# biagiom/spark-network-traffic-classifier

Hardware: NVIDIA H100
Metric: flow-records/sec fit+transform (higher is better)
Workload: dtype u8 bins / uint32 histograms / f64 split scoring (f32 records)

## Files before the change

include/b200flow.h:

```cpp
#ifndef B200FLOW_H
#define B200FLOW_H

#include <stdint.h>

#ifdef __cplusplus
extern "C" {
#endif

#define B200FLOW_OK            0
#define B200FLOW_ERR_ARG      -1
#define B200FLOW_ERR_CUDA     -2
#define B200FLOW_ERR_LIMIT    -3

#define B200FLOW_F32 0
#define B200FLOW_F64 1

#define B200FLOW_SRC_F32    0
#define B200FLOW_SRC_F64    1
#define B200FLOW_SRC_I32    2
#define B200FLOW_SRC_INDEX  3
#define B200FLOW_SRC_ONEHOT 4

typedef struct b200flow_slot {
    int32_t kind;
// ... 114 lines not shown
                        const uint32_t* node_counts, const uint32_t* left_counts,
                        const uint32_t* right_counts, int32_t C,
                        b200flow_node* nodes, uint64_t* node_mask, uint32_t* pool_counts,
                        int32_t* node_tree, int64_t pool_capacity,
                        int32_t* next_tree, uint32_t* next_nid, int32_t* next_node,
                        int32_t* next_parent, int32_t* child_slot, int64_t* counters, void* stream);

int b200flow_partition_level(const uint8_t* tp, int32_t tp_stride,
                             const void* ent, void* ent_out,
                             int32_t n_slots, const int64_t* seg_begin, const int64_t* seg_end,
                             const int64_t* chunk_off, int64_t n_chunks, int32_t chunk_rows,
                             const b200flow_split* split, int32_t* cursors, void* stream);

int b200flow_route_hist_config(int32_t F, int32_t m, int32_t n_bins, int32_t C,
                               int32_t rec_bytes , int32_t* chunk_rows, int32_t* m_pass);
int b200flow_route_hist_level(const uint8_t* tp, int32_t tp_stride, int32_t F,
                              const int32_t* field_desc ,
                              const void* ent, void* ent_out,
                              int32_t n_slots, const int64_t* seg_begin, const int64_t* seg_end,
                              const int64_t* chunk_off, const int64_t* n_chunks_dev ,
                              int64_t n_chunks_max ,
                              int32_t chunk_rows,
                              const b200flow_split* split, const int32_t* child_slot, int32_t* cursors,
                              void* chunk_scratch ,
                              const uint16_t* subset_next, int32_t m, int32_t n_bins, int32_t C,
                              uint32_t* hist_next, int32_t flags, void* stream);

int b200flow_packed_layout(int32_t F, const int32_t* feat_bins, int32_t C, int32_t* desc, int32_t* rec_bytes);
int b200flow_pack_records(const uint8_t* tp, int32_t tp_stride, int64_t n_rows, int32_t F, const int32_t* desc,
                          int32_t rec_bytes, uint32_t* packed, void* stream);

int b200flow_plan_route(int32_t n_slots, const b200flow_split* split, const int64_t* seg_begin, const int64_t* seg_end,
                        int32_t chunk_rows, const int32_t* slot_node, double* node_gain, int32_t* n_chunks,
                        int32_t* cursors , void* stream);

int b200flow_next_segments(int32_t n_next , const int64_t* n_next_dev ,
                           const int32_t* next_parent,
                           const int64_t* seg_begin, const int64_t* seg_end,
                           const int32_t* cursors, int64_t* next_begin, int64_t* next_end,
                           void* stream);

int b200flow_finalize_forest(int64_t n_nodes, const uint32_t* pool_counts, int32_t C,
                             double* leaf_prob, void* stream);

int b200flow_predict(const uint8_t* tp, int32_t tp_stride, int64_t n_rows,
                     const b200flow_node* nodes, const uint64_t* node_mask,
                     const double* leaf_prob, const uint32_t* pool_counts,
                     int32_t T, int32_t C, int32_t dt_mode,
                     const void* top_nodes , int32_t top_levels,
                     double* raw, double* prob, double* pred, void* stream);

int b200flow_build_top_nodes(const b200flow_node* nodes, const int32_t* node_tree, int64_t n_nodes, int32_t T,
                             int32_t top_levels, void* top, void* stream);

int b200flow_gather_rows(const void* src, int32_t row_bytes, const int32_t* idx, int64_t n_rows, void* out, void* stream);

int b200flow_confusion(const double* pred, const double* label, int64_t n_rows, int32_t C,
                       int64_t* cm, void* stream);

int b200flow_predict_grid_confusion(const uint8_t* tp, int32_t tp_stride, int32_t F, int64_t n_rows, const int32_t* mult,
                                    const b200flow_node* nodes, const uint64_t* node_mask, const double* leaf_prob,
                                    const uint32_t* pool_counts, int32_t T, int32_t C, int32_t dt_mode,
                                    const void* top_nodes, int32_t top_levels, const int32_t* tree_cuts_host,
                                    int32_t n_tree_cuts, const int32_t* depth_cuts_host, int32_t n_depth_cuts,
                                    int32_t cm_side, int32_t max_depth_cuts_per_launch, int64_t* cm, void* stream);
int b200flow_predict_grid_scores(const uint8_t* tp, int32_t tp_stride, int32_t F, int64_t n_rows,
                                 const b200flow_node* nodes, const uint64_t* node_mask, const double* leaf_prob,
                                 const uint32_t* pool_counts, int32_t T, int32_t C, int32_t dt_mode,
                                 const void* top_nodes, int32_t top_levels, const int32_t* tree_cuts_host,
                                 int32_t n_tree_cuts, const int32_t* depth_cuts_host, int32_t n_depth_cuts,
                                 int32_t max_depth_cuts_per_launch, double* scores, void* stream);

int b200flow_binary_counts_scratch(int32_t S, int64_t n, int64_t* scratch_bytes);
int b200flow_binary_counts(const double* scores, int64_t score_stride, const int32_t* pos, const int32_t* neg,
                           int64_t count_stride, int32_t S, int64_t n, void* scratch, int64_t scratch_bytes,
                           double* d_score, int64_t* d_pos, int64_t* d_neg, int64_t cap, int64_t* n_distinct,
                           int64_t* n_nan, void* stream);
int b200flow_binary_curve(const double* d_score, const int64_t* d_pos, const int64_t* d_neg, int64_t cap,
                          const int64_t* n_distinct, int32_t S, int32_t num_bins, double* auc, double* c_score,
                          int64_t* c_tp, int64_t* c_fp, int64_t* c_n, double* work, void* stream);

int b200flow_kmeans_assign(const double* x, int64_t n_rows, int32_t D, int64_t ld, const double* centers, int32_t k,
                           int32_t* cluster, double* dist, void* stream);
int b200flow_group_sums_chunks(int64_t row_offset, int64_t n_rows, int64_t* n_chunks);
int b200flow_group_sums(const double* values, int64_t ld, const int32_t* ids, int64_t n_rows, int32_t W, int32_t G,
                        int64_t row_offset, double* partials, int64_t* counts, void* stream);
int b200flow_group_sums_chain(const double* partials, int64_t n_chunks, int32_t G, int32_t W, double* totals, void* stream);
int b200flow_kmeans_row_keys(uint64_t seed, int64_t row_offset, int64_t n_rows, int64_t* keys, void* stream);
int b200flow_kmeans_select(uint64_t seed, int64_t row_offset, int64_t n_rows, int32_t step, const double* cost, int32_t k,
                           double sum_cost, uint8_t* flag, void* stream);
int b200flow_silhouette_rows(const double* x, int64_t n_rows, int32_t D, int64_t ld, const double* norms, const int32_t* cluster,
                             const double* Y, const double* psi, const int64_t* N, int32_t G, double* out, void* stream);

int b200flow_mlp_config(const int32_t* layers, int32_t n_layers, int64_t* n_params, int64_t* smem_bytes);
int b200flow_mlp_loss_grad(const void* x, int32_t x_dtype, int64_t n_rows, int64_t ld, const int32_t* labels,
                           const int32_t* layers, int32_t n_layers, const double* weights, int64_t row_offset,
                           double* partials, void* stream);
int b200flow_mlp_forward(const void* x, int32_t x_dtype, int64_t n_rows, int64_t ld, const int32_t* layers, int32_t n_layers,
                         const double* weights, double* raw, void* stream);

int b200flow_svc_config(int32_t D, int64_t K, int32_t* block_classes, int32_t* class_blocks, int64_t* smem_bytes);
int b200flow_svc_loss_grad(const void* x, int32_t x_dtype, int64_t n_rows, int64_t ld, int32_t D, const int32_t* labels,
                           const int32_t* positives, int64_t K, const double* inv_std, const double* weights,
                           int64_t row_offset, double* partials, void* stream);
int b200flow_svc_margins(const void* x, int32_t x_dtype, int64_t n_rows, int64_t ld, int32_t D, int64_t K,
                         const double* weights, double* raw, void* stream);
// ... 152 lines not shown
```

spark-network-traffic-classifier_b200/b200flow/_lib.py:

```python
import ctypes as C
import os

import numpy as np
import torch

_HERE = os.path.dirname(os.path.abspath(__file__))
LIB_PATH = os.path.join(_HERE, "libb200flow.so")

F32, F64 = 0, 1
SRC_F32, SRC_F64, SRC_I32, SRC_INDEX, SRC_ONEHOT = 0, 1, 2, 3, 4

SLOT_DTYPE = np.dtype([("kind", "<i4"), ("src_off", "<i4"), ("lut_off", "<i4"), ("lut_len", "<i4"),
                       ("hot", "<i4"), ("reserved", "<i4"), ("mean", "<f8"), ("scale", "<f8")])
SPLIT_DTYPE = np.dtype([("feat", "<i4"), ("kind", "<i4"), ("bin_thr", "<i4"), ("flags", "<i4"),
                        ("gain", "<f8"), ("impurity", "<f8"), ("mask", "<u8", (4,))])
NODE_DTYPE = np.dtype([("feat", "<i4"), ("kind_bin", "<i4"), ("left", "<i4"), ("nid", "<u4")])
assert SLOT_DTYPE.itemsize == 40 and SPLIT_DTYPE.itemsize == 64 and NODE_DTYPE.itemsize == 16


class B200FlowError(RuntimeError):
    pass


class UnsupportedParamError(B200FlowError, ValueError):
    """a parameter value MLlib accepts but the CUDA path does not implement (entropy impurity, maxBins > 256, ...): a
    ValueError, so the pyspark shim reports it as IllegalArgumentException; CUDA/runtime failures stay B200FlowError."""


_P, _I32, _I64, _U64, _F64 = C.c_void_p, C.c_int32, C.c_int64, C.c_uint64, C.c_double

_SIGNATURES = {
    "b200flow_category_counts": [_P, _I64, _I32, _I32, _I32, _P, _P],
    "b200flow_category_counts_multi": [_P, _I64, _I32, _I32, _P, _P, _P, _P],
    "b200flow_encode": [_P, _I64, _I32, _P, _I32, _P, _I32, _I32, _I32, _I32, _I32, _P, _I32, _P, _P, _P],
    "b200flow_sample_records": [_P, _I64, _I32, _P, _I32, _P, _I32, _U64, _U64, _I64, _P, _I64, _P, _P],
    "b200flow_encode_bins": [_P, _I64, _I32, _P, _I32, _P, _I32, _I32, _I32, _I32, _I32, _I32, _I32, _P, _P, _P, _I32, _P, _I32, _P, _P, _P],
    "b200flow_column_moments": [_P, _I32, _I64, _I32, _I64, _P, _P, _P, _P],
    "b200flow_sample_rows": [_P, _I32, _I64, _I32, _I64, _U64, _U64, _I64, _P, _I64, _P, _P],
    "b200flow_find_splits": [_P, _I64, _I32, _I32, _P, _I32, _P, _P, _P, _P],
    "b200flow_bin_rows": [_P, _I32, _I64, _I32, _I64, _P, _P, _P, _I32, _P, _P, _I32, _P, _P],
    "b200flow_dedup_rows": [_P, _I64, _I32, _I32, _P, _P, _I64, _P, _P, _P, _P, _P, _P, _P, _P],
    "b200flow_bag_weights": [_U64, _I32, _I64, _I64, _P, _P, _P, _P, _I64, _P, _P],
    "b200flow_group_rows": [_P, _I64, _I64, _P, _P, _P, _P, _P, _P],
    "b200flow_bag_count": [_P, _I32, _I64, _P, _P],
    "b200flow_bag_fill": [_P, _I32, _I64, _P, _P, _P],
    "b200flow_exclusive_scan_i32_to_i64": [_P, _I64, _P, _P, _P],
    "b200flow_feature_subsets": [_U64, _I32, _P, _P, _I32, _I32, _P, _P],
    "b200flow_hist_level": [_P, _I32, _I32, _P, _I32, _P, _P, _P, _I64, _I32, _P, _I32, _I32, _I32, _P, _P],
    "b200flow_score_level": [_P, _I32, _P, _I32, _I32, _I32, _P, _P, _I32, _I32, _I32, _F64, _P, _P, _P, _P, _P],
    "b200flow_grow_level": [_I32, _P, _P, _P, _P, _P, _P, _P, _I32, _P, _P, _P, _P, _I64, _P, _P, _P, _P, _P, _P, _P],
    "b200flow_route_hist_level": [_P, _I32, _I32, _P, _P, _P, _I32, _P, _P, _P, _P, _I64, _I32, _P, _P, _P, _P, _P, _I32, _I32,
                                  _I32, _P, _I32, _P],
    "b200flow_pack_records": [_P, _I32, _I64, _I32, _P, _I32, _P, _P],
    "b200flow_partition_level": [_P, _I32, _P, _P, _I32, _P, _P, _P, _I64, _I32, _P, _P, _P],
    "b200flow_plan_route": [_I32, _P, _P, _P, _I32, _P, _P, _P, _P, _P],
    "b200flow_next_segments": [_I32, _P, _P, _P, _P, _P, _P, _P, _P],
    "b200flow_finalize_forest": [_I64, _P, _I32, _P, _P],
    "b200flow_predict": [_P, _I32, _I64, _P, _P, _P, _P, _I32, _I32, _I32, _P, _I32, _P, _P, _P, _P],
    "b200flow_build_top_nodes": [_P, _P, _I64, _I32, _I32, _P, _P],
    "b200flow_gather_rows": [_P, _I32, _P, _I64, _P, _P],
    "b200flow_confusion": [_P, _P, _I64, _I32, _P, _P],
    "b200flow_predict_grid_confusion": [_P, _I32, _I32, _I64, _P, _P, _P, _P, _P, _I32, _I32, _I32, _P, _I32, _P, _I32, _P, _I32,
                                        _I32, _I32, _P, _P],
    "b200flow_predict_grid_scores": [_P, _I32, _I32, _I64, _P, _P, _P, _P, _I32, _I32, _I32, _P, _I32, _P, _I32, _P, _I32, _I32,
                                     _P],
    "b200flow_binary_counts": [_P, _I64, _P, _P, _I64, _I32, _I64, _P, _I64, _P, _P, _P, _I64, _P, _P, _P],
    "b200flow_binary_curve": [_P, _P, _P, _I64, _P, _I32, _I32, _P, _P, _P, _P, _P, _P, _P],
    "b200flow_kmeans_assign": [_P, _I64, _I32, _I64, _P, _I32, _P, _P, _P],
    "b200flow_group_sums": [_P, _I64, _P, _I64, _I32, _I32, _I64, _P, _P, _P],
    "b200flow_group_sums_chain": [_P, _I64, _I32, _I32, _P, _P],
    "b200flow_kmeans_row_keys": [_U64, _I64, _I64, _P, _P],
    "b200flow_kmeans_select": [_U64, _I64, _I64, _I32, _P, _I32, _F64, _P, _P],
    "b200flow_silhouette_rows": [_P, _I64, _I32, _I64, _P, _P, _P, _P, _P, _I32, _P, _P],
    "b200flow_mlp_loss_grad": [_P, _I32, _I64, _I64, _P, _P, _I32, _P, _I64, _P, _P],
    "b200flow_mlp_forward": [_P, _I32, _I64, _I64, _P, _I32, _P, _P, _P],
    "b200flow_svc_loss_grad": [_P, _I32, _I64, _I64, _I32, _P, _P, _I64, _P, _P, _I64, _P, _P],
    "b200flow_svc_margins": [_P, _I32, _I64, _I64, _I32, _I64, _P, _P, _P],
    "b200flow_linreg_loss_grad": [_P, _I32, _I64, _I64, _I32, _P, _P, _P, _F64, _F64, _P, _P, _F64, _I32, _I64, _P, _P],
    "b200flow_aft_loss_grad": [_P, _I32, _I64, _I64, _I32, _P, _P, _P, _P, _P, _P, _I64, _P, _P],
    "b200flow_glm_rows": [_P, _I32, _I64, _I64, _I32, _P, _P, _P, _P, _F64, _F64, _I32, _I32, _F64, _F64, _I32, _I64, _P, _P,
                          _P],
    "b200flow_isotonic_fit": [_P, _I32, _I64, _P, _I64, _P, _I64, _I64, _I32, _I64, _P, _I64, _P, _P, _P, _P, _P],
    "b200flow_isotonic_predict": [_P, _I32, _I64, _I64, _P, _P, _I64, _P, _P],
    "b200flow_fm_loss_grad": [_P, _I32, _I64, _I64, _I32, _I32, _P, _P, _I64, _P, _F64, _U64, _I64, _P, _P],
    "b200flow_fm_regression_loss_grad": [_P, _I32, _I64, _I64, _I32, _I32, _P, _P, _F64, _U64, _I64, _P, _P],
    "b200flow_fm_raw": [_P, _I32, _I64, _I64, _I32, _I32, _I64, _P, _P, _P],
    "b200flow_gmm_estep": [_P, _I64, _I32, _I64, _I32, _P, _P, _P, _I64, _P, _P, _P, _P],
    "b200flow_gmm_moments": [_P, _I64, _I32, _I64, _I32, _P, _I64, _P, _P],
    "b200flow_centered_gram": [_P, _I64, _I32, _I64, _P, _I64, _P, _P],
    "b200flow_weighted_centered_gram": [_P, _I64, _I32, _I64, _P, _P, _I64, _P, _P],
    "b200flow_pca_project": [_P, _I64, _I32, _I64, _P, _I32, _P, _P],
    "b200flow_distinct_values": [_P, _I64, _I32, _I64, _P, _P, _P, _P],
    "b200flow_dictionary_ids": [_P, _I64, _I64, _P, _I32, _P, _P],
    "b200flow_contingency_counts": [_P, _I64, _I32, _I64, _P, _I32, _P, _P, _I64, _P, _P],
    "b200flow_group_centered_moments": [_P, _I64, _I32, _I64, _P, _I32, _P, _P, _F64, _I64, _P, _P],
    "b200flow_gbt_hist_level": [_P, _I32, _P, _P, _I32, _P, _P, _P, _I64, _I32, _P, _I32, _I32, _P, _P],
    "b200flow_gbt_hist_level_classes": [_P, _I32, _P, _P, _I64, _P, _I32, _P, _P, _P, _I64, _I32, _P, _I32, _I32, _P, _P],
    "b200flow_gbt_score_level": [_P, _I32, _P, _I32, _I32, _P, _P, _I32, _I32, _I32, _I32, _I32, _F64, _P, _P, _P, _P, _P],
    "b200flow_gbt_leaf_values": [_I64, _P, _P, _P, _I32, _P, _P],
    "b200flow_gbt_update": [_P, _I32, _I32, _I64, _P, _P, _P, _I32, _I32, _I32, _P, _P, _P],
    "b200flow_gbt_update_classes": [_P, _I32, _I32, _I64, _I32, _P, _P, _P, _I32, _I32, _I32, _I32, _P, _P, _P],
    "b200flow_gbt_output": [_P, _I64, _P, _P, _P, _P],
    "b200flow_reg_labels": [_P, _I64, _P, _I32, _I32, _P, _P],
    "b200flow_reg_tree_weights": [_P, _I32, _I64, _P, _P],
    "b200flow_reg_grid": [_P, _I32, _I32, _P, _I64, _I32, _I32, _I32, _P, _P],
    "b200flow_reg_leaf_table": [_I64, _P, _I32, _I32, _P, _I32, _P],
    "b200flow_reg_divide": [_P, _I64, _F64, _P, _P],
    "b200flow_gbr_leaf_values": [_I64, _P, _P, _I32, _F64, _I32, _P, _P],
    "b200flow_gbr_update": [_P, _I32, _I32, _P, _I64, _P, _P, _P, _I32, _I32, _P, _P, _P, _P],
    "b200flow_reg_eval_max": [_P, _P, _I64, _I32, _F64, _P, _P],
    "b200flow_reg_eval_sums": [_P, _P, _I64, _I32, _F64, _I32, _I32, _I32, _I32, _P, _P],
    "b200flow_random_split": [_U64, _I64, _I64, _P, _I32, _P, _P],
# ... 161 lines not shown
```

spark-network-traffic-classifier_b200/b200flow/forest.py:

```python
import math
from dataclasses import dataclass

import numpy as np
import torch

from . import _lib
from ._lib import NODE_DTYPE, SPLIT_DTYPE, B200FlowError, UnsupportedParamError, call, ptr

import os as _os
CHUNK_ROWS = 2048
FUSED = True
TOP_LEVELS = int(_os.environ.get("B200FLOW_TOP_LEVELS", "8"))
DEDUP = True
_PIN = True
PROFILE = None


def _timed(name, fn, *args):
    if PROFILE is None:
        return call(fn, *args)
    e0, e1 = torch.cuda.Event(enable_timing=True), torch.cuda.Event(enable_timing=True)
    e0.record()
    call(fn, *args)
    e1.record()
# ... 141 lines not shown
        self.n, self.F = rec.shape[0], plan.n_out
        self.device = rec.device
        self.with_label = with_label and plan.label is not None

    def _thr_f32(self, arity_dev):
        if self.round_f32:
            return 1
        return 1 if all(s[0] in (_lib.SRC_F32, _lib.SRC_INDEX, _lib.SRC_ONEHOT) and s[5] == 0.0 and s[6] == 1.0 for s in self.plan.slots) else 0

    def sample(self, seed, keep, row_offset, sample, cap, n_s_dev):
        _, slots, lut_t, _ = self.plan._device_tables(self.device)
        call("b200flow_sample_records", ptr(self.rec), self.n, self.plan.schema.row_bytes, ptr(slots), self.F, ptr(lut_t), self.round_f32,
             seed, keep, int(row_offset), ptr(sample), cap, ptr(n_s_dev))

    def bin(self, thresholds, n_thr, arity_dev, mpb, bad, want_label_out=False):
        _, slots, lut_t, lut_total = self.plan._device_tables(self.device)
        stride = tp_stride(self.F)
        tp = torch.empty((self.n, stride), dtype=torch.uint8, device=self.device)
        loff, llo, lln = self.plan.label if self.with_label else (-1, 0, 0)
        lab = torch.empty(self.n, dtype=torch.int32, device=self.device) if (want_label_out and self.with_label) else None
        _timed("encode_bins", "b200flow_encode_bins", ptr(self.rec), self.n, self.plan.schema.row_bytes, ptr(slots), self.F, ptr(lut_t), lut_total,
               loff, llo, lln, int(self.plan.check_nan), self.round_f32, self._thr_f32(arity_dev), ptr(thresholds), ptr(n_thr), ptr(arity_dev), mpb, ptr(tp), stride,
               ptr(lab), ptr(bad))
        return tp, lab


class ForestModel:

    def __init__(self, T, C, F, arity, max_bins, thresholds, n_thr, nodes, node_mask, pool_counts, node_tree,
                 leaf_prob, node_gain, n_nodes, dt_mode):
        self.T, self.C, self.F, self.max_bins, self.dt_mode = T, C, F, max_bins, dt_mode
        self.arity = np.asarray(arity, np.int32)
        self.thresholds, self.n_thr = thresholds, n_thr
        self.nodes, self.node_mask, self.pool_counts = nodes, node_mask, pool_counts
        self.node_tree, self.leaf_prob, self.node_gain, self.n_nodes = node_tree, leaf_prob, node_gain, n_nodes
        self._arity_dev = _i32(self.arity, thresholds.device)

    def bin(self, x, labels=None):
        n, F = x.shape
        if F != self.F:
            raise ValueError("expected %d features, got %d" % (self.F, F))
        bad = torch.zeros(2, dtype=torch.int32, device=x.device)
        tp, _ = _DenseSource(x, labels).bin(self.thresholds, self.n_thr, self._arity_dev, self.max_bins, bad)
        return tp, bad[0:1]

    def _top_table(self):
        if TOP_LEVELS <= 0:
            return None, 0
        if getattr(self, "_top", None) is None:
            self._top = torch.zeros((self.T << TOP_LEVELS, 4), dtype=torch.int32, device=self.nodes.device)
            call("b200flow_build_top_nodes", ptr(self.nodes), ptr(self.node_tree), self.n_nodes, self.T, TOP_LEVELS, ptr(self._top))
        return self._top, TOP_LEVELS

    def predict_binned(self, tp, want_raw=True, want_prob=True):
        n = tp.shape[0]
        dev = tp.device
        raw = torch.empty((n, self.C), dtype=torch.float64, device=dev) if want_raw else None
        prob = torch.empty((n, self.C), dtype=torch.float64, device=dev) if want_prob else None
        pred = torch.empty(n, dtype=torch.float64, device=dev)
        top, K = self._top_table()
        _timed("predict", "b200flow_predict", ptr(tp), tp.shape[1], n, ptr(self.nodes), ptr(self.node_mask), ptr(self.leaf_prob),
             ptr(self.pool_counts), self.T, self.C, 1 if self.dt_mode else 0, ptr(top), K, ptr(raw), ptr(prob), ptr(pred))
        return raw, prob, pred

    def predict(self, x, want_raw=True, want_prob=True):
        tp, _ = self.bin(x)
        return self._predict_tp(tp, want_raw, want_prob)

    def predict_records(self, rec, plan, want_raw=True, want_prob=True, round_f32=False, want_label=False, on_invalid="ignore"):
        src = _RecordSource(rec, plan, round_f32, with_label=want_label)
        if src.F != self.F:
            raise ValueError("expected %d features, got %d" % (self.F, src.F))
        bad = torch.zeros(2, dtype=torch.int32, device=rec.device)
        tp, lab = src.bin(self.thresholds, self.n_thr, self._arity_dev, self.max_bins, bad, want_label_out=want_label)
        out = self._predict_tp(tp, want_raw, want_prob, bad if on_invalid == "error" else None)
        return out + (lab,)

    def _predict_tp(self, tp, want_raw=True, want_prob=True, bad=None):
        n = tp.shape[0]
        if not DEDUP or n == 0:
            if bad is not None and int(bad[1].item()):
                raise InvalidRowsError("%d NaN/null cells or unseen labels in the rows to transform" % int(bad[1].item()))
            return self.predict_binned(tp, want_raw, want_prob)
        tpu, uid, u_dev = dedup_rows(tp, self.F, sync=False)
        head = (torch.cat([u_dev, bad.to(torch.int64)]) if bad is not None else u_dev).cpu()
        if bad is not None and int(head[2]):
            raise InvalidRowsError("%d NaN/null cells or unseen labels in the rows to transform" % int(head[2]))
        U = int(head[0])
        raw_u, prob_u, pred_u = self.predict_binned(tpu[:U], want_raw, want_prob)

        def spread(src, width):
            if src is None:
                return None
            out = torch.empty((n, width) if width > 1 else (n,), dtype=torch.float64, device=tp.device)
            call("b200flow_gather_rows", ptr(src), 8 * width, ptr(uid), n, ptr(out))
            return out
        return spread(raw_u, self.C), spread(prob_u, self.C), spread(pred_u, 1)

    def grid_confusion(self, x_or_records, tree_cuts, depth_cuts, labels=None, plan=None, round_f32=False, cm_side=None,
                       group=None, max_depth_cuts_per_launch=0):
        from . import dist as bdist
        tree_cuts = np.ascontiguousarray(sorted(set(int(t) for t in tree_cuts)), np.int32)
        depth_cuts = np.ascontiguousarray(sorted(set(int(d) for d in depth_cuts)), np.int32)
        if plan is None:
            if labels is None:
                raise ValueError("grid_confusion: the dense path needs the labels")
            src = _DenseSource(x_or_records, labels)
        else:
            if plan.label is None:
                raise ValueError("grid_confusion: the encode plan has no label column (EncodePlan.set_label)")
            src = _RecordSource(x_or_records, plan, round_f32)
        if src.F != self.F:
            raise ValueError("expected %d features, got %d" % (self.F, src.F))
        S = max(self.C, int(cm_side or 0))
        dev = src.device
# ... 561 lines not shown
```

spark-network-traffic-classifier_b200/b200flow/gbt_regression.py:

```python
from dataclasses import dataclass

import numpy as np
import torch

from . import _lib
from . import forest as fr
from . import gbt as bg
from . import regression as rg
from ._lib import call, ptr

LOSSES = {"squared": 0, "absolute": 1}


@dataclass
class GBTRegressorParams:
    max_iter: int = 20
    step_size: float = 0.1
    max_depth: int = 5
    max_bins: int = 32
    min_instances_per_node: int = 1
    min_info_gain: float = 0.0
    subsampling_rate: float = 1.0
    feature_subset_strategy: str = "all"
    seed: int = 0
    loss: str = "squared"


def residual_exponent(max_abs):
    if max_abs > 2.0 ** rg.E_MAX:
        raise ValueError("a boosting residual of magnitude %r is beyond the regression trainer's range (|r| <= 2^%d)"
                         % (max_abs, rg.E_MAX))
    return rg.label_grid(max_abs, 2)[0]


class GBTRegressionModel:

    def __init__(self, forest, tree_weights, stats, E, S, S2):
        self.forest = forest
        self.T, self.F = forest.T, forest.F
        self.tree_weights = list(tree_weights)
        self.stats, self.E, self.S, self.S2 = stats, list(E), S, S2

    @property
    def n_nodes(self):
        return self.forest.n_nodes

    def predict(self, x):
        raw, _, _ = self.forest.predict(x, want_raw=True, want_prob=False)
        return raw.reshape(-1)

    def predict_records(self, rec, plan, round_f32=False, on_invalid="ignore"):
        raw, _, _, _ = self.forest.predict_records(rec, plan, want_raw=True, want_prob=False, round_f32=round_f32,
                                                   on_invalid=on_invalid)
        return raw.reshape(-1)

    def _prefix(self, k):
        fo = self.forest
        pre = fr.ForestModel(k, 1, fo.F, fo.arity, fo.max_bins, fo.thresholds, fo.n_thr, fo.nodes, fo.node_mask, None,
                             fo.node_tree, fo.leaf_prob, fo.node_gain, fo.n_nodes, dt_mode=False)
        top, _ = fo._top_table()
        if top is not None:
            pre._top = top
        return pre

    def prefix_predictions(self, x):
        tp, _ = self.forest.bin(x)
        n = tp.shape[0]
        uid = None
        if fr.DEDUP and n > 0:
            tp, uid, _ = fr.dedup_rows(tp, self.F)
        for k in range(1, self.T + 1):
            raw, _, _ = self._prefix(k).predict_binned(tp, want_raw=True, want_prob=False)
            if uid is None:
                yield raw.reshape(-1)
                continue
            out = torch.empty(n, dtype=torch.float64, device=tp.device)
            call("b200flow_gather_rows", ptr(raw.contiguous()), 8, ptr(uid), n, ptr(out))
            yield out

    def evaluate_each_iteration(self, x, y, loss, group=None):
        from .metrics import regression_metrics
        if loss not in LOSSES:
            raise ValueError("loss must be one of %s, got %r" % (sorted(LOSSES), loss))
        key = "mse" if loss == "squared" else "mae"
        y = y.to(torch.float64).reshape(-1).contiguous()
        return [regression_metrics(y, p, group=group)[key] for p in self.prefix_predictions(x)]

    def export(self):
        return bg.export_pool(self.forest, self.stats)

    def leaf_values(self, ex=None):
        ex = self.export() if ex is None else ex
        sh = self.S - np.asarray(self.E, np.int64)[ex["tree"]]
        with np.errstate(all="ignore"):
            return (ex["stats"][:, 1].astype(np.float64) * np.ldexp(1.0, -sh)) / ex["stats"][:, 0].astype(np.float64)

    def feature_importances(self):
        ex = self.export()
        v = np.zeros(self.F)
        sel = ex["is_leaf"] == 0
        np.add.at(v, ex["feat"][sel], ex["gain"][sel] * ex["stats"][sel, 0].astype(np.float64))
        return v / v.sum() if v.sum() > 0 else v


def fit_gbt_regressor(x, y, arity, params, row_offset=0, group=None):
    from . import dist as bdist
    import torch.distributed as dist
    _lib.require_cuda()
    p = params
    if not (0 <= p.max_depth <= 30):
        raise ValueError("maxDepth must be in [0, 30], got %d" % p.max_depth)
    if int(p.max_iter) < 1:
        raise ValueError("maxIter must be >= 1, got %d" % p.max_iter)
    if not (0.0 < p.step_size <= 1.0):
        raise ValueError("stepSize must be in (0, 1], got %r" % p.step_size)
# ... 108 lines not shown
```

spark-network-traffic-classifier_b200/csrc/predict.cu:

```cuda
#include <stdlib.h>

#include "common.cuh"

namespace b200flow {


__global__ void __launch_bounds__(256) build_top_kernel(const int4* __restrict__ nodes, const int32_t* __restrict__ node_tree,
                                                        int64_t n_nodes, int K, int4* top) {
    const int64_t i = (int64_t)blockIdx.x * blockDim.x + threadIdx.x;
    if (i >= n_nodes) return;
    const int4 nd = nodes[i];
    if ((uint32_t)nd.w < (1u << K)) top[((int64_t)node_tree[i] << K) + nd.w] = nd;
}

template <int kPredRows>
__global__ void __launch_bounds__(128) predict_kernel(const uint8_t* __restrict__ tp, int stride, int64_t n,
                                                      const b200flow_node* __restrict__ nodes,
                                                      const unsigned long long* __restrict__ node_mask,
                                                      const double* __restrict__ leaf_prob,
                                                      const uint32_t* __restrict__ pool_counts, int T, int C, int dt_mode,
                                                      const int4* __restrict__ top, int K,
                                                      double* raw, double* prob, double* pred) {
    extern __shared__ __align__(16) uint8_t sm[];
    const int bd = blockDim.x, tid = threadIdx.x;
    const int words = stride / 4;
    uint32_t* binw = (uint32_t*)sm;
    double* votes = (double*)(sm + (size_t)kPredRows * words * bd * 4);
    const int topn = top ? (1 << K) : 0;
    int4* topbuf = (int4*)(votes + (size_t)kPredRows * C * bd);
    auto stage_top = [&](int t, int buf) {
        if (t < T) for (int i = tid; i < topn; i += bd) cp_async16(topbuf + (size_t)buf * topn + i, top + ((int64_t)t << K) + i);
        cp_async_commit();
    };
    for (int64_t base = (int64_t)blockIdx.x * bd * kPredRows; base < n; base += (int64_t)gridDim.x * bd * kPredRows) {
        int64_t row[kPredRows]; bool live[kPredRows];
#pragma unroll
        for (int r = 0; r < kPredRows; ++r) {
            row[r] = base + (int64_t)r * bd + tid; live[r] = row[r] < n;
            uint32_t* bw = binw + (size_t)r * words * bd;
            if (live[r]) {
                const uint4* src = (const uint4*)(tp + row[r] * stride);
                for (int q = 0; q < words / 4; ++q) {
                    const uint4 v = ld_stream_u4(src + q);
                    bw[(4 * q + 0) * bd + tid] = v.x; bw[(4 * q + 1) * bd + tid] = v.y;
                    bw[(4 * q + 2) * bd + tid] = v.z; bw[(4 * q + 3) * bd + tid] = v.w;
                }
            }
            for (int k = 0; k < C; ++k) votes[((size_t)r * C + k) * bd + tid] = 0.0;
        }
        const uint32_t* bw0 = binw + tid;
        const int4* nodes4 = (const int4*)nodes;
        if (top) stage_top(0, 0);
        for (int t = 0; t < T; ++t) {
            const int4* tb = topbuf + (size_t)(t & 1) * topn;
            if (top) {
                cp_async_wait_all();
                __syncthreads();
                stage_top(t + 1, (t + 1) & 1);
            }
            int idx[kPredRows]; uint32_t nid[kPredRows]; int4 nd[kPredRows];
#pragma unroll
            for (int r = 0; r < kPredRows; ++r) { idx[r] = t; nid[r] = 1u; nd[r] = top ? tb[1] : __ldg(nodes4 + t); if (!live[r]) nd[r].x = -1; }
            while (true) {
                bool any = false;
#pragma unroll
                for (int r = 0; r < kPredRows; ++r) {
                    if (nd[r].x >= 0) {
                        const int f = nd[r].x;
                        const int bin = (bw0[(r * words + (f >> 2)) * bd] >> ((f & 3) * 8)) & 0xff;
                        const int right = nd[r].y < 65536 ? (bin > nd[r].y)
                                                          : !((node_mask[(int64_t)idx[r] * 4 + (bin >> 6)] >> (bin & 63)) & 1ull);
                        idx[r] = nd[r].z + right;
                        nid[r] = 2u * nid[r] + (uint32_t)right;
                        any = true;
                    }
                }
                if (!any) break;
#pragma unroll
                for (int r = 0; r < kPredRows; ++r)
                    if (nd[r].x >= 0) nd[r] = nid[r] < (uint32_t)topn ? tb[nid[r]] : __ldg(nodes4 + idx[r]);
            }
#pragma unroll
            for (int r = 0; r < kPredRows; ++r) {
                if (!live[r]) continue;
                double* vt = votes + (size_t)r * C * bd + tid;
                if (dt_mode) { for (int k = 0; k < C; ++k) vt[k * bd] += (double)pool_counts[(int64_t)idx[r] * C + k]; }
                else { for (int k = 0; k < C; ++k) vt[k * bd] += leaf_prob[(int64_t)idx[r] * C + k]; }
            }
        }
#pragma unroll
        for (int r = 0; r < kPredRows; ++r) {
            if (!live[r]) continue;
            const double* vt = votes + (size_t)r * C * bd + tid;
            double s = 0.0; int arg = 0; double best = vt[0];
            for (int k = 0; k < C; ++k) { const double v = vt[k * bd]; s += v; if (v > best) { best = v; arg = k; } }
            for (int k = 0; k < C; ++k) {
                const double v = vt[k * bd];
                if (raw) raw[row[r] * C + k] = v;
                if (prob) prob[row[r] * C + k] = s != 0.0 ? v / s : 0.0;
            }
            pred[row[r]] = (double)arg;
        }
        if (top) { cp_async_wait_all(); __syncthreads(); }
    }
}

__global__ void __launch_bounds__(256) gather_rows_kernel(const uint32_t* __restrict__ src, int words, const int32_t* __restrict__ idx,
                                                          int64_t n, uint32_t* out) {
    const int64_t total = n * words;
    for (int64_t e = (int64_t)blockIdx.x * blockDim.x + threadIdx.x; e < total; e += (int64_t)gridDim.x * blockDim.x) {
        const int64_t r = e / words; const int w = (int)(e - r * words);
        out[e] = __ldg(src + (int64_t)idx[r] * words + w);
    }
}

__global__ void __launch_bounds__(256) confusion_kernel(const double* __restrict__ pred, const double* __restrict__ label,
                                                        int64_t n, int C, unsigned long long* cm, int use_smem) {
    extern __shared__ uint32_t sh_cm[];
    if (use_smem) { for (int i = threadIdx.x; i < C * C; i += blockDim.x) sh_cm[i] = 0; __syncthreads(); }
    for (int64_t i = (int64_t)blockIdx.x * blockDim.x + threadIdx.x; i < n; i += (int64_t)gridDim.x * blockDim.x) {
        const int l = (int)label[i], p = (int)pred[i];
        if (l >= 0 && l < C && p >= 0 && p < C) {
            if (use_smem) atomicAdd(&sh_cm[l * C + p], 1u); else atomicAdd(&cm[l * C + p], 1ull);
        }
    }
    if (use_smem) {
        __syncthreads();
        for (int i = threadIdx.x; i < C * C; i += blockDim.x) if (sh_cm[i]) atomicAdd(&cm[i], (unsigned long long)sh_cm[i]);
    }
}

constexpr int kGridMaxTreeCuts = 256;
constexpr int kGridMaxDepthCuts = 31;
struct GridCuts { int32_t tree[kGridMaxTreeCuts]; int32_t depth[kGridMaxDepthCuts]; };

template <bool kScores>
__global__ void __launch_bounds__(128) predict_grid_kernel(const uint8_t* __restrict__ tp, int stride, int F, int64_t n,
                                                           const int32_t* __restrict__ mult,
                                                           const b200flow_node* __restrict__ nodes,
                                                           const unsigned long long* __restrict__ node_mask,
                                                           const double* __restrict__ leaf_prob,
                                                           const uint32_t* __restrict__ pool_counts, int C, int dt_mode,
                                                           const int4* __restrict__ top, int K, const GridCuts cuts, int I,
                                                           int J, int j0, int jn, int L, unsigned long long* cm, int use_smem,
                                                           double* scores) {
    extern __shared__ __align__(16) uint8_t sm[];
    const int bd = blockDim.x, tid = threadIdx.x;
    const int words = stride / 4;
    uint32_t* binw = (uint32_t*)sm;
    double* votes = (double*)(sm + (size_t)words * bd * 4);
    const int topn = top ? (1 << K) : 0;
    int4* topbuf = (int4*)(votes + (size_t)jn * C * bd);
    unsigned long long* sh_cm = (unsigned long long*)(topbuf + 2 * topn);
    const int T = cuts.tree[I - 1];
    const int cm_cells = I * jn * L * L;
    if (use_smem) { for (int i = tid; i < cm_cells; i += bd) sh_cm[i] = 0ull; __syncthreads(); }
    auto stage_top = [&](int t, int buf) {
// ... 132 lines not shown
    const int words = row_bytes / 4;
    const uint32_t* src = (const uint32_t*)(rows + rb0 * row_bytes);
    uint32_t* dst = (uint32_t*)(out + blk_off[blockIdx.x] * row_bytes);
    for (int64_t i = threadIdx.x; i < (int64_t)tot * words; i += blockDim.x) {
        int r = (int)(i / words), wd = (int)(i - (int64_t)r * words);
        dst[i] = src[(int64_t)src_of[r] * words + wd];
    }
}

}

using namespace b200flow;

extern "C" int b200flow_build_top_nodes(const b200flow_node* nodes, const int32_t* node_tree, int64_t n_nodes, int32_t T,
                                        int32_t top_levels, void* top, void* stream) {
    B2F_REQUIRE(nodes && node_tree && top && T > 0 && top_levels >= 1 && top_levels <= 10 && ((uintptr_t)top & 15) == 0, "build_top_nodes: bad arguments");
    if (n_nodes <= 0) return B200FLOW_OK;
    build_top_kernel<<<(unsigned)((n_nodes + 255) / 256), 256, 0, (cudaStream_t)stream>>>((const int4*)nodes, node_tree, n_nodes, top_levels, (int4*)top);
    return check_launch("build_top_nodes");
}

extern "C" int b200flow_predict(const uint8_t* tp, int32_t tp_stride, int64_t n_rows, const b200flow_node* nodes,
                                const uint64_t* node_mask, const double* leaf_prob, const uint32_t* pool_counts, int32_t T,
                                int32_t C, int32_t dt_mode, const void* top_nodes, int32_t top_levels,
                                double* raw, double* prob, double* pred, void* stream) {
    if (n_rows <= 0) return B200FLOW_OK;
    B2F_REQUIRE(tp && nodes && pred && T > 0 && C > 0 && (tp_stride & 15) == 0, "predict: bad arguments");
    B2F_REQUIRE(dt_mode ? pool_counts != nullptr : leaf_prob != nullptr, "predict: missing leaf payload");
    B2F_REQUIRE(((uintptr_t)tp & 15) == 0, "predict: tp must be 16-byte aligned");
    B2F_REQUIRE(!top_nodes || (top_levels >= 1 && top_levels <= 10 && ((uintptr_t)top_nodes & 15) == 0), "predict: bad top table");
    static int rows_per_thread = -1;
    if (rows_per_thread < 0) { const char* e = getenv("B200FLOW_PRED_ROWS"); rows_per_thread = (e && atoi(e) == 4) ? 4 : 2; }
    const int kPredRows = rows_per_thread;
    int bd = 128;
    size_t per_thread = ((size_t)tp_stride + (size_t)C * 8) * kPredRows;
    while (bd > 32 && per_thread * bd > 96 * 1024) bd >>= 1;
    size_t smem = per_thread * bd + (top_nodes ? (size_t)2 * 16 * ((size_t)1 << top_levels) : 0);
    B2F_REQUIRE(smem <= 200 * 1024, "predict: too many classes/features for shared memory");
    int grid = grid_for(n_rows, bd * kPredRows, kNumSMs * 16);
    cudaError_t e;
    if (kPredRows == 4) {
        e = cudaFuncSetAttribute(predict_kernel<4>, cudaFuncAttributeMaxDynamicSharedMemorySize, (int)smem);
        if (e == cudaSuccess) predict_kernel<4><<<grid, bd, smem, (cudaStream_t)stream>>>(tp, tp_stride, n_rows, nodes, (const unsigned long long*)node_mask, leaf_prob,
                                                                                          pool_counts, T, C, dt_mode, (const int4*)top_nodes, top_levels, raw, prob, pred);
    } else {
        e = cudaFuncSetAttribute(predict_kernel<2>, cudaFuncAttributeMaxDynamicSharedMemorySize, (int)smem);
        if (e == cudaSuccess) predict_kernel<2><<<grid, bd, smem, (cudaStream_t)stream>>>(tp, tp_stride, n_rows, nodes, (const unsigned long long*)node_mask, leaf_prob,
                                                                                          pool_counts, T, C, dt_mode, (const int4*)top_nodes, top_levels, raw, prob, pred);
    }
    if (e != cudaSuccess) { set_error("predict: %s", cudaGetErrorString(e)); return B200FLOW_ERR_CUDA; }
    return check_launch("predict");
}

extern "C" int b200flow_gather_rows(const void* src, int32_t row_bytes, const int32_t* idx, int64_t n_rows, void* out, void* stream) {
    if (n_rows <= 0) return B200FLOW_OK;
    B2F_REQUIRE(src && idx && out && row_bytes > 0 && (row_bytes & 3) == 0, "gather_rows: bad arguments");
    const int words = row_bytes / 4;
    gather_rows_kernel<<<grid_for(n_rows * words, 256 * 4, kNumSMs * 8), 256, 0, (cudaStream_t)stream>>>((const uint32_t*)src, words, idx, n_rows, (uint32_t*)out);
    return check_launch("gather_rows");
}

extern "C" int b200flow_confusion(const double* pred, const double* label, int64_t n_rows, int32_t C, int64_t* cm, void* stream) {
    if (n_rows <= 0) return B200FLOW_OK;
    B2F_REQUIRE(pred && label && cm && C > 0 && C <= 1024, "confusion: bad arguments");
    int use_smem = (size_t)C * C * 4 <= 64 * 1024;
    size_t smem = use_smem ? (size_t)C * C * 4 : 0;
    if (smem > 48 * 1024) cudaFuncSetAttribute(confusion_kernel, cudaFuncAttributeMaxDynamicSharedMemorySize, (int)smem);
    int grid = grid_for(n_rows, 256 * 8, kNumSMs * 4);
    confusion_kernel<<<grid, 256, smem, (cudaStream_t)stream>>>(pred, label, n_rows, C, (unsigned long long*)cm, use_smem);
    return check_launch("confusion");
}

template <bool kScores>
static int predict_grid_launch(const char* what, const uint8_t* tp, int32_t tp_stride, int32_t F, int64_t n_rows, const int32_t* mult,
                               const b200flow_node* nodes, const uint64_t* node_mask, const double* leaf_prob,
                               const uint32_t* pool_counts, int32_t T, int32_t C, int32_t dt_mode,
                               const void* top_nodes, int32_t top_levels, const int32_t* tree_cuts_host,
                               int32_t n_tree_cuts, const int32_t* depth_cuts_host, int32_t n_depth_cuts,
                               int32_t cm_side, int32_t max_depth_cuts_per_launch, int64_t* cm, double* scores, void* stream) {
    const int I = n_tree_cuts, J = n_depth_cuts, L = cm_side;
    B2F_REQUIRE(tree_cuts_host && depth_cuts_host && I >= 1 && I <= kGridMaxTreeCuts && J >= 1 && J <= kGridMaxDepthCuts,
                "%s: 1..%d tree cuts and 1..%d depth cuts", what, kGridMaxTreeCuts, kGridMaxDepthCuts);
    GridCuts cuts;
    for (int i = 0; i < I; ++i) {
        B2F_REQUIRE(tree_cuts_host[i] >= 1 && tree_cuts_host[i] <= T && (i == 0 || tree_cuts_host[i] > tree_cuts_host[i - 1]),
                    "%s: tree cuts must ascend strictly within [1, %d]", what, T);
        cuts.tree[i] = tree_cuts_host[i];
    }
    for (int j = 0; j < J; ++j) {
        B2F_REQUIRE(depth_cuts_host[j] >= 0 && depth_cuts_host[j] <= 30 && (j == 0 || depth_cuts_host[j] > depth_cuts_host[j - 1]),
                    "%s: depth cuts must ascend strictly within [0, 30]", what);
        cuts.depth[j] = depth_cuts_host[j];
    }
    if (n_rows <= 0) return B200FLOW_OK;
    if (kScores) B2F_REQUIRE(tp && nodes && scores && T > 0 && C >= 2 && F >= 0 && F < tp_stride && (tp_stride & 15) == 0,
                             "predict_grid_scores: bad arguments (C >= 2: the score is votes[1])");
    else B2F_REQUIRE(tp && mult && nodes && cm && T > 0 && C > 0 && L >= C && F >= 0 && F < tp_stride && (tp_stride & 15) == 0,
                     "predict_grid_confusion: bad arguments");
    B2F_REQUIRE(dt_mode ? pool_counts != nullptr : leaf_prob != nullptr, "%s: missing leaf payload", what);
    B2F_REQUIRE(((uintptr_t)tp & 15) == 0, "%s: tp must be 16-byte aligned", what);
    B2F_REQUIRE(!top_nodes || (top_levels >= 1 && top_levels <= 10 && ((uintptr_t)top_nodes & 15) == 0),
                "%s: bad top table", what);
    const size_t kBudget = 200 * 1024;
    const size_t top_bytes = top_nodes ? (size_t)2 * 16 * ((size_t)1 << top_levels) : 0;
    const int want = max_depth_cuts_per_launch > 0 && max_depth_cuts_per_launch < J ? max_depth_cuts_per_launch : J;
    auto cuts_that_fit = [&](int bd) -> int {
// ... 77 lines not shown
```

Measured before the change: 153.9 million.

## Predict forest with per-tree compact layout staged through shared memory

Adds a compact per-tree layout, built once and cached: each tree's nodes are renumbered locally and packed into 8-byte records with threshold/feature bits, categorical masks and leaf vote payloads stored inline. A new predict kernel stages each tree's block into shared memory with cp.async double buffering while rows' bins sit in shared memory, then traverses all trees per row and accumulates votes in registers when C is small. This replaces the old global-memory node walk with a top-node table, aiming to cut scattered global loads during inference. It adds a one-time layout build cost and relies on near-full shared memory with one block per SM, which may limit occupancy.

```diff
diff --git a/include/b200flow.h b/include/b200flow.h
--- a/include/b200flow.h
+++ b/include/b200flow.h
@@ -190,6 +190,15 @@
 
 int b200flow_build_top_nodes(const b200flow_node* nodes, const int32_t* node_tree, int64_t n_nodes, int32_t T,
                              int32_t top_levels, void* top, void* stream);
+
+int b200flow_forest_layout_size(const b200flow_node* nodes, const int32_t* node_tree, int64_t n_nodes, int32_t T, int32_t C,
+                                int32_t* scratch, int64_t* tree_off, void* stream);
+int b200flow_build_forest_layout(const b200flow_node* nodes, const uint64_t* node_mask, const double* leaf_prob,
+                                 const uint32_t* pool_counts, const int32_t* node_tree, int64_t n_nodes, int32_t T, int32_t C,
+                                 int32_t dt_mode, const int32_t* scratch, const int64_t* tree_off, uint64_t* layout, void* stream);
+
+int b200flow_predict_forest(const uint8_t* tp, int32_t tp_stride, int32_t F, int64_t n_rows, const uint64_t* layout,
+                            const int64_t* tree_off, int32_t T, int32_t C, double* raw, double* prob, double* pred, void* stream);
 
 int b200flow_gather_rows(const void* src, int32_t row_bytes, const int32_t* idx, int64_t n_rows, void* out, void* stream);
 
diff --git a/spark-network-traffic-classifier_b200/b200flow/_lib.py b/spark-network-traffic-classifier_b200/b200flow/_lib.py
--- a/spark-network-traffic-classifier_b200/b200flow/_lib.py
+++ b/spark-network-traffic-classifier_b200/b200flow/_lib.py
@@ -58,6 +58,9 @@
     "b200flow_finalize_forest": [_I64, _P, _I32, _P, _P],
     "b200flow_predict": [_P, _I32, _I64, _P, _P, _P, _P, _I32, _I32, _I32, _P, _I32, _P, _P, _P, _P],
     "b200flow_build_top_nodes": [_P, _P, _I64, _I32, _I32, _P, _P],
+    "b200flow_forest_layout_size": [_P, _P, _I64, _I32, _I32, _P, _P, _P],
+    "b200flow_build_forest_layout": [_P, _P, _P, _P, _P, _I64, _I32, _I32, _I32, _P, _P, _P, _P],
+    "b200flow_predict_forest": [_P, _I32, _I32, _I64, _P, _P, _I32, _I32, _P, _P, _P, _P],
     "b200flow_gather_rows": [_P, _I32, _P, _I64, _P, _P],
     "b200flow_confusion": [_P, _P, _I64, _I32, _P, _P],
     "b200flow_predict_grid_confusion": [_P, _I32, _I32, _I64, _P, _P, _P, _P, _P, _I32, _I32, _I32, _P, _I32, _P, _I32, _P, _I32,
diff --git a/spark-network-traffic-classifier_b200/b200flow/forest.py b/spark-network-traffic-classifier_b200/b200flow/forest.py
--- a/spark-network-traffic-classifier_b200/b200flow/forest.py
+++ b/spark-network-traffic-classifier_b200/b200flow/forest.py
@@ -217,15 +217,31 @@
             call("b200flow_build_top_nodes", ptr(self.nodes), ptr(self.node_tree), self.n_nodes, self.T, TOP_LEVELS, ptr(self._top))
         return self._top, TOP_LEVELS
 
+    def _forest_layout(self):
+        if getattr(self, "_layout", None) is None:
+            dev = self.nodes.device
+            scratch = torch.empty(2 * self.n_nodes + 4 * self.T, dtype=torch.int32, device=dev)
+            tree_off = torch.empty(self.T + 1, dtype=torch.int64, device=dev)
+            call("b200flow_forest_layout_size", ptr(self.nodes), ptr(self.node_tree), self.n_nodes, self.T, self.C, ptr(scratch),
+                 ptr(tree_off))
+            layout = torch.empty(max(int(tree_off[self.T].item()), 2), dtype=torch.int64, device=dev)
+            call("b200flow_build_forest_layout", ptr(self.nodes), ptr(self.node_mask), ptr(self.leaf_prob), ptr(self.pool_counts),
+                 ptr(self.node_tree), self.n_nodes, self.T, self.C, 1 if self.dt_mode else 0, ptr(scratch), ptr(tree_off),
+                 ptr(layout))
+            self._layout = (layout, tree_off)
+        return self._layout
+
     def predict_binned(self, tp, want_raw=True, want_prob=True):
         n = tp.shape[0]
         dev = tp.device
         raw = torch.empty((n, self.C), dtype=torch.float64, device=dev) if want_raw else None
         prob = torch.empty((n, self.C), dtype=torch.float64, device=dev) if want_prob else None
         pred = torch.empty(n, dtype=torch.float64, device=dev)
-        top, K = self._top_table()
-        _timed("predict", "b200flow_predict", ptr(tp), tp.shape[1], n, ptr(self.nodes), ptr(self.node_mask), ptr(self.leaf_prob),
-             ptr(self.pool_counts), self.T, self.C, 1 if self.dt_mode else 0, ptr(top), K, ptr(raw), ptr(prob), ptr(pred))
+        if n == 0:
+            return raw, prob, pred
+        layout, tree_off = self._forest_layout()
+        _timed("predict", "b200flow_predict_forest", ptr(tp), tp.shape[1], self.F, n, ptr(layout), ptr(tree_off), self.T, self.C,
+               ptr(raw), ptr(prob), ptr(pred))
         return raw, prob, pred
 
     def predict(self, x, want_raw=True, want_prob=True):
diff --git a/spark-network-traffic-classifier_b200/b200flow/gbt_regression.py b/spark-network-traffic-classifier_b200/b200flow/gbt_regression.py
--- a/spark-network-traffic-classifier_b200/b200flow/gbt_regression.py
+++ b/spark-network-traffic-classifier_b200/b200flow/gbt_regression.py
@@ -61,6 +61,7 @@
         top, _ = fo._top_table()
         if top is not None:
             pre._top = top
+        pre._layout = fo._forest_layout()
         return pre
 
     def prefix_predictions(self, x):
diff --git a/spark-network-traffic-classifier_b200/csrc/predict.cu b/spark-network-traffic-classifier_b200/csrc/predict.cu
--- a/spark-network-traffic-classifier_b200/csrc/predict.cu
+++ b/spark-network-traffic-classifier_b200/csrc/predict.cu
@@ -1,4 +1,5 @@
 #include <stdlib.h>
+#include <type_traits>
 
 #include "common.cuh"
 
@@ -103,6 +104,212 @@
         }
         if (top) { cp_async_wait_all(); __syncthreads(); }
     }
+}
+
+constexpr uint32_t kLayoutLeaf = 1u << 31, kLayoutCat = 1u << 30;
+constexpr int kLayoutCatWords = 5;
+constexpr int kLayoutRankBlock = 1024, kLayoutRankPer = 4;
+constexpr int kVoteBatch = 8;
+constexpr int kPredForestRegC = 8;
+constexpr int kPredForestRegThreads = 896;
+
+__device__ __forceinline__ unsigned long long block_exclusive_scan_u64(unsigned long long v, unsigned long long* sh,
+                                                                      unsigned long long* total) {
+    const unsigned long long inc = warp_inclusive_scan(v);
+    if (lane_id() == 31) sh[warp_id()] = inc;
+    __syncthreads();
+    if (warp_id() == 0) {
+        const unsigned long long w = sh[lane_id()];
+        const unsigned long long winc = warp_inclusive_scan(w);
+        sh[lane_id()] = winc - w;
+        if (lane_id() == 31) sh[32] = winc;
+    }
+    __syncthreads();
+    const unsigned long long res = inc - v + sh[warp_id()];
+    *total = sh[32];
+    __syncthreads();
+    return res;
+}
+
+__global__ void __launch_bounds__(kLayoutRankBlock) layout_rank_kernel(const int4* __restrict__ nodes,
+                                                                        const int32_t* __restrict__ node_tree, int64_t n, int C,
+                                                                        int32_t* local, int32_t* ord, int32_t* cnt, int32_t* words) {
+    __shared__ unsigned long long sh[33];
+    const int t = blockIdx.x;
+    constexpr unsigned long long kOne = 1ull, kLeafOne = 1ull << 21, kCatOne = 1ull << 42, kField = (1ull << 21) - 1;
+    int64_t base_n = 0, base_l = 0, base_c = 0;
+    for (int64_t c0 = 0; c0 < n; c0 += (int64_t)kLayoutRankBlock * kLayoutRankPer) {
+        const int64_t i0 = c0 + (int64_t)threadIdx.x * kLayoutRankPer;
+        unsigned long long inc[kLayoutRankPer], v = 0;
+#pragma unroll
+        for (int j = 0; j < kLayoutRankPer; ++j) {
+            inc[j] = 0;
+            const int64_t i = i0 + j;
+            if (i < n && node_tree[i] == t) {
+                const int4 nd = __ldg(nodes + i);
+                inc[j] = kOne | (nd.x < 0 ? kLeafOne : ((uint32_t)nd.y >= 65536u ? kCatOne : 0ull));
+            }
+            v += inc[j];
+        }
+        unsigned long long total;
+        unsigned long long pre = block_exclusive_scan_u64(v, sh, &total);
+#pragma unroll
+        for (int j = 0; j < kLayoutRankPer; ++j) {
+            if (inc[j]) {
+                const int64_t i = i0 + j;
+                local[i] = (int32_t)(base_n + (pre & kField));
+                ord[i] = (int32_t)((inc[j] & kLeafOne) ? base_l + ((pre >> 21) & kField)
+                                                       : base_c + ((pre >> 42) & kField));
+            }
+            pre += inc[j];
+        }
+        base_n += total & kField; base_l += (total >> 21) & kField; base_c += (total >> 42) & kField;
+    }
+    if (threadIdx.x == 0) {
+        cnt[3 * t] = (int32_t)base_n; cnt[3 * t + 1] = (int32_t)base_l; cnt[3 * t + 2] = (int32_t)base_c;
+        const int64_t w = base_n + base_l * C + base_c * kLayoutCatWords;
+        words[t] = (int32_t)((w + 1) & ~1ll);
+    }
+}
+
+__global__ void __launch_bounds__(256) layout_fill_kernel(const int4* __restrict__ nodes,
+                                                          const unsigned long long* __restrict__ node_mask,
+                                                          const double* __restrict__ leaf_prob,
+                                                          const uint32_t* __restrict__ pool_counts,
+                                                          const int32_t* __restrict__ node_tree, int64_t n, int T, int C,
+                                                          int dt_mode, const int32_t* __restrict__ local,
+                                                          const int32_t* __restrict__ ord, const int32_t* __restrict__ cnt,
+                                                          const int64_t* __restrict__ tree_off, uint2* layout) {
+    const int64_t i = (int64_t)blockIdx.x * blockDim.x + threadIdx.x;
+    if (i >= n) return;
+    const int t = node_tree[i];
+    if (t < 0 || t >= T) return;
+    uint2* blk = layout + tree_off[t];
+    const int4 nd = nodes[i];
+    const uint32_t n_t = (uint32_t)cnt[3 * t], c_t = (uint32_t)cnt[3 * t + 2];
+    uint2 rec;
+    if (nd.x < 0) {
+        const uint32_t vo = n_t + c_t * kLayoutCatWords + (uint32_t)ord[i] * (uint32_t)C;
+        rec = make_uint2(kLayoutLeaf, vo);
+        double* v = (double*)(blk + vo);
+        if (dt_mode) { for (int k = 0; k < C; ++k) v[k] = (double)pool_counts[i * C + k]; }
+        else { for (int k = 0; k < C; ++k) v[k] = leaf_prob[i * C + k]; }
+    } else if ((uint32_t)nd.y >= 65536u) {
+        const uint32_t co = n_t + (uint32_t)ord[i] * kLayoutCatWords;
+        rec = make_uint2((uint32_t)nd.x | kLayoutCat, co);
+        blk[co] = make_uint2((uint32_t)local[nd.z], 0u);
+        unsigned long long* m = (unsigned long long*)(blk + co + 1);
+        for (int q = 0; q < 4; ++q) m[q] = node_mask ? node_mask[i * 4 + q] : 0ull;
+    } else {
+        const uint32_t thr = (uint32_t)nd.y < 255u ? (uint32_t)nd.y : 255u;
+        rec = make_uint2((uint32_t)nd.x | (thr << 16), (uint32_t)local[nd.z]);
+    }
+    blk[local[i]] = rec;
+}
+
+template <int kRegC>
+__global__ void __launch_bounds__(kRegC ? kPredForestRegThreads : 1024, 1)
+predict_forest_kernel(const uint8_t* __restrict__ tp, int stride, int fwords, int64_t n, const uint2* __restrict__ layout,
+                      const int64_t* __restrict__ tree_off, int T, int C, int cap, double* raw, double* prob, double* pred) {
+    extern __shared__ __align__(16) uint8_t sm[];
+    const int bd = blockDim.x, tid = threadIdx.x;
+    uint32_t* binw = (uint32_t*)sm;
+    double* votes = (double*)(sm + (size_t)fwords * bd * 4);
+    uint2* tbuf = (uint2*)(votes + (kRegC ? 0 : (size_t)C * bd));
+    auto stage = [&](int t, int buf) {
+        if (t >= 0) {
+            const int64_t o = tree_off[t];
+            const int64_t w = tree_off[t + 1] - o < cap ? tree_off[t + 1] - o : cap;
+            const uint4* src = (const uint4*)(layout + o);
+            uint4* dst = (uint4*)(tbuf + (size_t)buf * cap);
+            for (int i = tid; i < (int)(w >> 1); i += bd) cp_async16(dst + i, src + i);
+        }
+        cp_async_commit();
+    };
+    const int64_t round_rows = (int64_t)gridDim.x * bd;
+    const uint8_t* bb = (const uint8_t*)(binw + tid);
+    double* vt = votes + tid;
+    int g = 0;
+    if ((int64_t)blockIdx.x * bd < n) stage(0, 0);
+    for (int64_t base = (int64_t)blockIdx.x * bd; base < n; base += round_rows) {
+        const int64_t row = base + tid;
+        const bool live = row < n;
+        if (live) {
+            const uint4* src = (const uint4*)(tp + row * stride);
+            for (int q = 0; q < fwords / 4; ++q) {
+                const uint4 v = ld_stream_u4(src + q);
+                binw[(4 * q + 0) * bd + tid] = v.x; binw[(4 * q + 1) * bd + tid] = v.y;
+                binw[(4 * q + 2) * bd + tid] = v.z; binw[(4 * q + 3) * bd + tid] = v.w;
+            }
+        }
+        double acc[kRegC > 0 ? kRegC : 1];
+#pragma unroll
+        for (int k = 0; k < (kRegC > 0 ? kRegC : 1); ++k) acc[k] = 0.0;
+        if (!kRegC) for (int k = 0; k < C; ++k) vt[k * bd] = 0.0;
+        for (int t = 0; t < T; ++t, ++g) {
+            cp_async_wait_all();
+            __syncthreads();
+            stage(t + 1 < T ? t + 1 : (base + round_rows < n ? 0 : -1), (g + 1) & 1);
+            const uint2* tb = tbuf + (size_t)(g & 1) * cap;
+            const uint2* gb = layout + tree_off[t];
+            const bool whole = tree_off[t + 1] - tree_off[t] <= cap;
+            auto walk = [&](auto whole_tag) {
+                constexpr bool kWhole = decltype(whole_tag)::value;
+                auto word = [&](uint32_t o) -> uint2 { return (kWhole || o < (uint32_t)cap) ? tb[o] : __ldg(gb + o); };
+                if (!live) return;
+                uint2 nd = word(0);
+                while (!(nd.x & kLayoutLeaf)) {
+                    const uint32_t f = nd.x & 0xffff;
+                    const uint32_t bin = bb[(f & ~3u) * bd + (f & 3u)];
+                    uint32_t next;
+                    if (nd.x & kLayoutCat) {
+                        const uint2 m = word(nd.y + 1 + (bin >> 6));
+                        next = word(nd.y).x + !((((bin & 32) ? m.y : m.x) >> (bin & 31)) & 1u);
+                    } else {
+                        next = nd.y + (bin > ((nd.x >> 16) & 0xff));
+                    }
+                    nd = word(next);
+                }
+                if (kRegC) {
+#pragma unroll
+                    for (int k = 0; k < kRegC; ++k)
+                        if (k < C) { const uint2 w = word(nd.y + k); acc[k] += __hiloint2double((int)w.y, (int)w.x); }
+                } else {
+                    for (int k0 = 0; k0 < C; k0 += kVoteBatch) {
+                        uint2 w[kVoteBatch];
+#pragma unroll
+                        for (int j = 0; j < kVoteBatch; ++j) if (k0 + j < C) w[j] = word(nd.y + k0 + j);
+#pragma unroll
+                        for (int j = 0; j < kVoteBatch; ++j)
+                            if (k0 + j < C) vt[(k0 + j) * bd] += __hiloint2double((int)w[j].y, (int)w[j].x);
+                    }
+                }
+            };
+            if (whole) walk(std::integral_constant<bool, true>()); else walk(std::integral_constant<bool, false>());
+        }
+        if (!live) continue;
+        if (kRegC) {
+            double s = 0.0; int arg = 0; double best = acc[0];
+#pragma unroll
+            for (int k = 0; k < kRegC; ++k) if (k < C) { s += acc[k]; if (acc[k] > best) { best = acc[k]; arg = k; } }
+#pragma unroll
+            for (int k = 0; k < kRegC; ++k) if (k < C) {
+                if (raw) raw[row * C + k] = acc[k];
+                if (prob) prob[row * C + k] = s != 0.0 ? acc[k] / s : 0.0;
+            }
+            pred[row] = (double)arg;
+        } else {
+            double s = 0.0; int arg = 0; double best = vt[0];
+            for (int k = 0; k < C; ++k) { const double v = vt[k * bd]; s += v; if (v > best) { best = v; arg = k; } }
+            for (int k = 0; k < C; ++k) {
+                const double v = vt[k * bd];
+                if (raw) raw[row * C + k] = v;
+                if (prob) prob[row * C + k] = s != 0.0 ? v / s : 0.0;
+            }
+            pred[row] = (double)arg;
+        }
+    }
+    cp_async_wait_all();
 }
 
 __global__ void __launch_bounds__(256) gather_rows_kernel(const uint32_t* __restrict__ src, int words, const int32_t* __restrict__ idx,
@@ -341,6 +548,66 @@
     return check_launch("predict");
 }
 
+extern "C" int b200flow_forest_layout_size(const b200flow_node* nodes, const int32_t* node_tree, int64_t n_nodes, int32_t T,
+                                           int32_t C, int32_t* scratch, int64_t* tree_off, void* stream) {
+    B2F_REQUIRE(nodes && node_tree && scratch && tree_off && T > 0 && C > 0 && n_nodes >= T, "forest_layout_size: bad arguments");
+    B2F_REQUIRE(n_nodes * ((int64_t)C + kLayoutCatWords + 1) < ((int64_t)1 << 31), "forest_layout_size: forest too large for 32-bit offsets");
+    cudaStream_t st = (cudaStream_t)stream;
+    int32_t* local = scratch; int32_t* ord = scratch + n_nodes; int32_t* cnt = ord + n_nodes; int32_t* words = cnt + 3 * (int64_t)T;
+    layout_rank_kernel<<<T, kLayoutRankBlock, 0, st>>>((const int4*)nodes, node_tree, n_nodes, C, local, ord, cnt, words);
+    const int rc = check_launch("forest_layout_size");
+    if (rc) return rc;
+    return b200flow_exclusive_scan_i32_to_i64(words, T, tree_off, tree_off + T, stream);
+}
+
+extern "C" int b200flow_build_forest_layout(const b200flow_node* nodes, const uint64_t* node_mask, const double* leaf_prob,
+                                            const uint32_t* pool_counts, const int32_t* node_tree, int64_t n_nodes, int32_t T,
+                                            int32_t C, int32_t dt_mode, const int32_t* scratch, const int64_t* tree_off,
+                                            uint64_t* layout, void* stream) {
+    B2F_REQUIRE(nodes && node_tree && scratch && tree_off && layout && T > 0 && C > 0 && n_nodes >= T && ((uintptr_t)layout & 15) == 0,
+                "build_forest_layout: bad arguments");
+    B2F_REQUIRE(dt_mode ? pool_counts != nullptr : leaf_prob != nullptr, "build_forest_layout: missing leaf payload");
+    const int32_t* local = scratch; const int32_t* ord = scratch + n_nodes; const int32_t* cnt = ord + n_nodes;
+    layout_fill_kernel<<<(unsigned)((n_nodes + 255) / 256), 256, 0, (cudaStream_t)stream>>>(
+        (const int4*)nodes, (const unsigned long long*)node_mask, leaf_prob, pool_counts, node_tree, n_nodes, T, C, dt_mode,
+        local, ord, cnt, tree_off, (uint2*)layout);
+    return check_launch("build_forest_layout");
+}
+
+constexpr size_t kPredForestSmem = 227 * 1024;
+
+extern "C" int b200flow_predict_forest(const uint8_t* tp, int32_t tp_stride, int32_t F, int64_t n_rows, const uint64_t* layout,
+                                       const int64_t* tree_off, int32_t T, int32_t C, double* raw, double* prob, double* pred,
+                                       void* stream) {
+    if (n_rows <= 0) return B200FLOW_OK;
+    B2F_REQUIRE(tp && layout && tree_off && pred && T > 0 && C > 0 && F > 0 && F < 65536 && F <= tp_stride && (tp_stride & 15) == 0,
+                "predict_forest: bad arguments");
+    B2F_REQUIRE(((uintptr_t)tp & 15) == 0 && ((uintptr_t)layout & 15) == 0, "predict_forest: tp and layout must be 16-byte aligned");
+    const bool reg = C <= kPredForestRegC;
+    const int fwords = (F + 15) / 16 * 4;
+    const size_t row_bytes = (size_t)fwords * 4 + (reg ? 0 : (size_t)C * 8);
+    const int64_t max_bd = reg ? kPredForestRegThreads : 1024;
+    int64_t bd = (int64_t)(kPredForestSmem / 2 / row_bytes) / 32 * 32;
+    if (bd > max_bd) bd = max_bd;
+    if (bd < 32) bd = 32;
+    B2F_REQUIRE((size_t)bd * row_bytes + 16 <= kPredForestSmem, "predict_forest: too many classes/features for shared memory");
+    const int64_t rounds = (n_rows + (int64_t)kNumSMs * bd - 1) / ((int64_t)kNumSMs * bd);
+    const int64_t want = (n_rows + (int64_t)kNumSMs * rounds - 1) / ((int64_t)kNumSMs * rounds);
+    bd = (want + 31) / 32 * 32 < bd ? (want + 31) / 32 * 32 : bd;
+    const int grid = grid_for(n_rows, (int)bd, kNumSMs);
+    const size_t rows_smem = (size_t)bd * row_bytes;
+    const int cap = (int)((kPredForestSmem - rows_smem) / 16) & ~1;
+    const size_t smem = rows_smem + (size_t)2 * cap * 8;
+    const void* fn = reg ? (const void*)predict_forest_kernel<kPredForestRegC> : (const void*)predict_forest_kernel<0>;
+    cudaError_t e = cudaFuncSetAttribute(fn, cudaFuncAttributeMaxDynamicSharedMemorySize, (int)smem);
+    if (e != cudaSuccess) { set_error("predict_forest: %s", cudaGetErrorString(e)); return B200FLOW_ERR_CUDA; }
+    if (reg) predict_forest_kernel<kPredForestRegC><<<grid, (int)bd, smem, (cudaStream_t)stream>>>(tp, tp_stride, fwords, n_rows,
+                                                                  (const uint2*)layout, tree_off, T, C, cap, raw, prob, pred);
+    else predict_forest_kernel<0><<<grid, (int)bd, smem, (cudaStream_t)stream>>>(tp, tp_stride, fwords, n_rows,
+                                                                  (const uint2*)layout, tree_off, T, C, cap, raw, prob, pred);
+    return check_launch("predict_forest");
+}
+
 extern "C" int b200flow_gather_rows(const void* src, int32_t row_bytes, const int32_t* idx, int64_t n_rows, void* out, void* stream) {
     if (n_rows <= 0) return B200FLOW_OK;
     B2F_REQUIRE(src && idx && out && row_bytes > 0 && (row_bytes & 3) == 0, "gather_rows: bad arguments");
```

Measured after the change: 159.4 million, median of 6. 1.04x the previous value.
